# kan-bayashi/ParallelWaveGAN

Hardware: AMD Instinct MI355X
Metric: HiFi-GAN V1 22.05 kHz generator inference RTF^-1 (audio samples/s) (higher is better)
Workload: dtype f32; 1 GPU; HiFi-GAN V1 generator fwd, LJSpeech 22.05 kHz, B16 x 800 mel frames per GPU, fp32, random init; global_batch=16, parallelism=replicas x1

## Files before the change

### include/pwg_kernels.h

```cpp
#ifndef PWG_KERNELS_H_
#define PWG_KERNELS_H_

#include <stddef.h>
#include <stdint.h>

#ifdef __cplusplus
extern "C" {
#endif

typedef enum pwg_status {
  PWG_OK = 0,
  PWG_ERR_BAD_SHAPE = -1,
  PWG_ERR_UNSUPPORTED = -2,
  PWG_ERR_LAUNCH = -3,
  PWG_ERR_NULL = -4,
  PWG_ERR_WORKSPACE = -5
} pwg_status;

const char* pwg_last_error(void);
int pwg_abi_version(void);
int pwg_target_arch(void);

int pwg_prof_enable(int on);
int pwg_prof_reset(void);
// ... 48 lines not shown
  const float* g;
  float* scale;
  float* fwd;
  float* bwd;
  pwg_conv1d_desc desc;
} pwg_bank_item;
size_t pwg_weight_bank_table_bytes(int32_t n_items);
int pwg_weight_bank_build(const pwg_bank_item* items, int32_t n_items, void* table_host, size_t table_bytes,
                          int32_t* info);
int pwg_weight_bank_prepare(const void* table_dev, const int32_t* info, int32_t with_bwd, void* stream);

size_t pwg_conv1d_backward_data_workspace_floats(const pwg_conv1d_desc* d);
int pwg_conv1d_backward_data(const pwg_conv1d_desc* d, const float* dy, const float* w_packed_bwd,
                             const float* x, const float* accum, float* dx, float* workspace,
                             size_t workspace_floats, void* stream);
size_t pwg_conv1d_backward_weight_workspace_floats(const pwg_conv1d_desc* d);
int pwg_conv1d_backward_weight(const pwg_conv1d_desc* d, const float* x, const float* dy, float* dw,
                               float* db, float* workspace, size_t workspace_floats, void* stream);

size_t pwg_conv1d_backward_weight_wn_workspace_floats(const pwg_conv1d_desc* d);
int pwg_conv1d_backward_weight_wn(const pwg_conv1d_desc* d, const float* x, const float* dy, const float* v,
                                  const float* g, float* dv, float* dg, float* db, float* workspace,
                                  size_t workspace_floats, void* stream);

int pwg_conv1d_num_tile_configs(void);
int pwg_conv1d_forward_cfg(const pwg_conv1d_desc* d, const float* x, const float* w_packed,
                           const float* bias, const float* add1, const float* add2, float* y,
                           int32_t tile_config, int32_t use_dma, void* stream);

int pwg_conv1d_bf16_supported(const pwg_conv1d_desc* d);
size_t pwg_conv1d_bf16_packed_weight_bytes(const pwg_conv1d_desc* d);
int pwg_conv1d_bf16_pack_weight(const pwg_conv1d_desc* d, const float* w, const float* scale, void* w_packed,
                                void* stream);
int pwg_conv1d_bf16_forward(const pwg_conv1d_desc* d, const float* x, const void* w_packed, const float* bias,
                            const float* add1, const float* add2, float* y, float* workspace, size_t workspace_floats,
                            void* stream);
int pwg_conv1d_bf16_forward_cfg(const pwg_conv1d_desc* d, const float* x, const void* w_packed, const float* bias,
                                const float* add1, const float* add2, float* y, int32_t mfma_shape, void* stream);

int pwg_conv1d_split_supported(const pwg_conv1d_desc* d);
size_t pwg_conv1d_split_packed_weight_bytes(const pwg_conv1d_desc* d);
int pwg_conv1d_split_pack_weight(const pwg_conv1d_desc* d, const float* w, const float* scale, void* w_packed,
                                 void* stream);
int pwg_conv1d_split_forward(const pwg_conv1d_desc* d, const float* x, const void* w_packed, const float* bias,
                             const float* add1, const float* add2, float* y, float* workspace, size_t workspace_floats,
                             void* stream);
int pwg_conv1d_split_forward_cfg(const pwg_conv1d_desc* d, const float* x, const void* w_packed, const float* bias,
                                 const float* add1, const float* add2, float* y, int32_t mfma_shape, int32_t tile_mode,
                                 void* stream);
int pwg_conv1d_split_step_form(const pwg_conv1d_desc* d);
int pwg_conv1d_split_forward_step(const pwg_conv1d_desc* d, const float* x, const void* w_packed, const float* bias,
                                  const float* add1, const float* add2, float* y, int32_t mfma_shape, int32_t tile_mode,
                                  int32_t step_form, void* stream);

int pwg_convtr1d_split_supported(const pwg_conv1d_desc* d);
size_t pwg_convtr1d_split_packed_weight_bytes(const pwg_conv1d_desc* d);
int pwg_convtr1d_split_pack_weight(const pwg_conv1d_desc* d, const float* w, const float* scale, void* w_packed,
                                   void* stream);
int pwg_convtr1d_split_forward(const pwg_conv1d_desc* d, const float* x, const void* w_packed, const float* bias,
                               const float* add1, const float* add2, float* y, float* workspace,
                               size_t workspace_floats, void* stream);
int pwg_convtr1d_split_forward_cfg(const pwg_conv1d_desc* d, const float* x, const void* w_packed, const float* bias,
                                   const float* add1, const float* add2, float* y, int32_t mfma_shape,
                                   int32_t tile_mode, void* stream);

int pwg_conv1d_stream_supported(const pwg_conv1d_desc* d);
size_t pwg_conv1d_stream_hist_floats(const pwg_conv1d_desc* d);
int pwg_conv1d_stream_forward(const pwg_conv1d_desc* d, const float* x, const float* hist_in, float* hist_out,
                              const float* w_packed, const float* bias, const float* add1, const float* add2, float* y,
                              void* stream);

int pwg_conv1d_stream_bf16_supported(const pwg_conv1d_desc* d);
int pwg_conv1d_stream_bf16_forward(const pwg_conv1d_desc* d, const float* x, const float* hist_in, float* hist_out,
                                   const void* w_packed_bf16, const float* bias, const float* add1,
                                   const float* add2, float* y, void* stream);

int pwg_conv1d_stream_delayed_supported(const pwg_conv1d_desc* d, int32_t delay1, int32_t delay2);
int pwg_conv1d_stream_delayed_forward(const pwg_conv1d_desc* d, const float* x, const float* hist_in, float* hist_out,
                                      const float* w_packed, const float* bias, const float* add1,
                                      const float* add1_hist_in, float* add1_hist_out, int32_t delay1, const float* add2,
                                      const float* add2_hist_in, float* add2_hist_out, int32_t delay2, int32_t valid_lo,
                                      int32_t valid_hi, float* y, void* stream);

int pwg_conv1d_stream_bf16_delayed_supported(const pwg_conv1d_desc* d, int32_t delay1, int32_t delay2);
int pwg_conv1d_stream_bf16_delayed_forward(const pwg_conv1d_desc* d, const float* x, const float* hist_in,
                                           float* hist_out, const void* w_packed_bf16, const float* bias,
                                           const float* add1, const float* add1_hist_in, float* add1_hist_out,
                                           int32_t delay1, const float* add2, const float* add2_hist_in,
                                           float* add2_hist_out, int32_t delay2, int32_t valid_lo, int32_t valid_hi,
                                           float* y, void* stream);

int pwg_conv1d_stream_slots_forward(const pwg_conv1d_desc* d, const float* x, const float* hist_in, float* hist_out,
                                    const float* w_packed, const float* bias, const float* add1,
                                    const float* add1_hist_in, float* add1_hist_out, int32_t delay1, const float* add2,
                                    const float* add2_hist_in, float* add2_hist_out, int32_t delay2, const int32_t* slots,
                                    int32_t rate, int32_t delay, float* y, void* stream);
int pwg_conv1d_stream_slots_forward_bf16(const pwg_conv1d_desc* d, const float* x, const float* hist_in, float* hist_out,
                                         const void* w_packed_bf16, const float* bias, const float* add1,
                                         const float* add1_hist_in, float* add1_hist_out, int32_t delay1,
                                         const float* add2, const float* add2_hist_in, float* add2_hist_out,
                                         int32_t delay2, const int32_t* slots, int32_t rate, int32_t delay, float* y,
                                         void* stream);

int pwg_conv1d_stream_mirrored_supported(const pwg_conv1d_desc* d);
int pwg_conv1d_stream_mirrored_forward(const pwg_conv1d_desc* d, const float* x, const float* hist_in, float* hist_out,
                                       const float* w_packed, const float* bias, float* y, int32_t in_lo, int32_t in_hi,
// ... 325 lines not shown
```

### parallelwavegan_amd/_lib.py

```python
import ctypes
import os

_HERE = os.path.dirname(os.path.abspath(__file__))
LIB_PATH = os.environ.get("PWG_KERNEL_LIB") or os.path.join(_HERE, "libpwgkernels.so")

PWG_ACT_NONE, PWG_ACT_LEAKY_RELU, PWG_ACT_TANH, PWG_ACT_RELU = 0, 1, 2, 3
PWG_PAD_ZERO, PWG_PAD_REFLECT, PWG_PAD_REPLICATE = 0, 1, 2
ABI_VERSION = 15
SPECTRAL_NORM_SCRATCH_FLOATS = 257


class ConvDesc(ctypes.Structure):

    _fields_ = [
        ("batch", ctypes.c_int32),
        ("c_in", ctypes.c_int32),
        ("c_out", ctypes.c_int32),
        ("t_in", ctypes.c_int32),
        ("t_out", ctypes.c_int32),
        ("width", ctypes.c_int32),
        ("kernel", ctypes.c_int32),
        ("stride", ctypes.c_int32),
        ("dilation", ctypes.c_int32),
        ("pad_left", ctypes.c_int32),
# ... 59 lines not shown
        ("a", ctypes.c_void_p),
        ("b", ctypes.c_void_p),
        ("da", ctypes.c_void_p),
        ("db", ctypes.c_void_p),
        ("n", ctypes.c_int64),
        ("mode", ctypes.c_int32),
        ("slot", ctypes.c_int32),
        ("scale", ctypes.c_float),
        ("c", ctypes.c_float),
    ]


RED_MAX_ITEMS = 64

_lib = None
_vp = ctypes.c_void_p
_i32 = ctypes.c_int32
_i64 = ctypes.c_int64
_f32 = ctypes.c_float

SIGNATURES = {
    "pwg_last_error": (ctypes.c_char_p, []),
    "pwg_abi_version": (ctypes.c_int, []),
    "pwg_target_arch": (ctypes.c_int, []),
    "pwg_debug_poison_lds": (ctypes.c_int, [ctypes.c_int]),
    "pwg_set_concurrency_hint": (ctypes.c_float, [ctypes.c_float]),
    "pwg_prof_enable": (ctypes.c_int, [ctypes.c_int]),
    "pwg_prof_reset": (ctypes.c_int, []),
    "pwg_prof_num_kernels": (ctypes.c_int, []),
    "pwg_prof_get": (ctypes.c_int, [_i32, ctypes.c_char_p, ctypes.c_size_t, ctypes.POINTER(ctypes.c_double),
                                    ctypes.POINTER(ctypes.c_int64), ctypes.POINTER(ctypes.c_double),
                                    ctypes.POINTER(ctypes.c_double)]),
    "pwg_conv1d_packed_weight_floats": (ctypes.c_size_t, [ctypes.POINTER(ConvDesc)]),
    "pwg_conv1d_pack_weight": (ctypes.c_int, [ctypes.POINTER(ConvDesc), _vp, _vp, _vp, _vp]),
    "pwg_conv1d_forward_workspace_floats": (ctypes.c_size_t, [ctypes.POINTER(ConvDesc)]),
    "pwg_conv1d_forward": (ctypes.c_int, [ctypes.POINTER(ConvDesc), _vp, _vp, _vp, _vp, _vp, _vp, _vp, ctypes.c_size_t,
                                          _vp]),
    "pwg_conv1d_bf16_supported": (ctypes.c_int, [ctypes.POINTER(ConvDesc)]),
    "pwg_conv1d_bf16_packed_weight_bytes": (ctypes.c_size_t, [ctypes.POINTER(ConvDesc)]),
    "pwg_conv1d_bf16_pack_weight": (ctypes.c_int, [ctypes.POINTER(ConvDesc), _vp, _vp, _vp, _vp]),
    "pwg_conv1d_bf16_forward": (ctypes.c_int, [ctypes.POINTER(ConvDesc), _vp, _vp, _vp, _vp, _vp, _vp, _vp, ctypes.c_size_t,
                                               _vp]),
    "pwg_conv1d_bf16_forward_cfg": (ctypes.c_int, [ctypes.POINTER(ConvDesc), _vp, _vp, _vp, _vp, _vp, _vp, _i32, _vp]),
    "pwg_conv1d_split_supported": (ctypes.c_int, [ctypes.POINTER(ConvDesc)]),
    "pwg_conv1d_split_packed_weight_bytes": (ctypes.c_size_t, [ctypes.POINTER(ConvDesc)]),
    "pwg_conv1d_split_pack_weight": (ctypes.c_int, [ctypes.POINTER(ConvDesc), _vp, _vp, _vp, _vp]),
    "pwg_conv1d_split_forward": (ctypes.c_int, [ctypes.POINTER(ConvDesc), _vp, _vp, _vp, _vp, _vp, _vp, _vp,
                                                ctypes.c_size_t, _vp]),
    "pwg_conv1d_split_forward_cfg": (ctypes.c_int, [ctypes.POINTER(ConvDesc), _vp, _vp, _vp, _vp, _vp, _vp, _i32, _i32,
                                                    _vp]),
    "pwg_conv1d_split_step_form": (ctypes.c_int, [ctypes.POINTER(ConvDesc)]),
    "pwg_conv1d_split_forward_step": (ctypes.c_int, [ctypes.POINTER(ConvDesc), _vp, _vp, _vp, _vp, _vp, _vp, _i32, _i32,
                                                     _i32, _vp]),
    "pwg_convtr1d_split_supported": (ctypes.c_int, [ctypes.POINTER(ConvDesc)]),
    "pwg_convtr1d_split_packed_weight_bytes": (ctypes.c_size_t, [ctypes.POINTER(ConvDesc)]),
    "pwg_convtr1d_split_pack_weight": (ctypes.c_int, [ctypes.POINTER(ConvDesc), _vp, _vp, _vp, _vp]),
    "pwg_convtr1d_split_forward": (ctypes.c_int, [ctypes.POINTER(ConvDesc), _vp, _vp, _vp, _vp, _vp, _vp, _vp,
                                                  ctypes.c_size_t, _vp]),
    "pwg_convtr1d_split_forward_cfg": (ctypes.c_int, [ctypes.POINTER(ConvDesc), _vp, _vp, _vp, _vp, _vp, _vp, _i32, _i32,
                                                      _vp]),
    "pwg_conv1d_stream_supported": (ctypes.c_int, [ctypes.POINTER(ConvDesc)]),
    "pwg_conv1d_stream_hist_floats": (ctypes.c_size_t, [ctypes.POINTER(ConvDesc)]),
    "pwg_conv1d_stream_forward": (ctypes.c_int, [ctypes.POINTER(ConvDesc), _vp, _vp, _vp, _vp, _vp, _vp, _vp, _vp, _vp]),
    "pwg_conv1d_stream_bf16_supported": (ctypes.c_int, [ctypes.POINTER(ConvDesc)]),
    "pwg_conv1d_stream_bf16_forward": (ctypes.c_int, [ctypes.POINTER(ConvDesc), _vp, _vp, _vp, _vp, _vp, _vp, _vp, _vp,
                                                      _vp]),
    "pwg_conv1d_stream_delayed_supported": (ctypes.c_int, [ctypes.POINTER(ConvDesc), _i32, _i32]),
    "pwg_conv1d_stream_delayed_forward": (ctypes.c_int, [ctypes.POINTER(ConvDesc), _vp, _vp, _vp, _vp, _vp, _vp, _vp, _vp,
                                                         _i32, _vp, _vp, _vp, _i32, _i32, _i32, _vp, _vp]),
    "pwg_conv1d_stream_bf16_delayed_supported": (ctypes.c_int, [ctypes.POINTER(ConvDesc), _i32, _i32]),
    "pwg_conv1d_stream_bf16_delayed_forward": (ctypes.c_int, [ctypes.POINTER(ConvDesc), _vp, _vp, _vp, _vp, _vp, _vp, _vp,
                                                              _vp, _i32, _vp, _vp, _vp, _i32, _i32, _i32, _vp, _vp]),
    "pwg_conv1d_stream_slots_forward": (ctypes.c_int, [ctypes.POINTER(ConvDesc), _vp, _vp, _vp, _vp, _vp, _vp, _vp, _vp,
                                                       _i32, _vp, _vp, _vp, _i32, _vp, _i32, _i32, _vp, _vp]),
    "pwg_conv1d_stream_slots_forward_bf16": (ctypes.c_int, [ctypes.POINTER(ConvDesc), _vp, _vp, _vp, _vp, _vp, _vp, _vp,
                                                            _vp, _i32, _vp, _vp, _vp, _i32, _vp, _i32, _i32, _vp, _vp]),
    "pwg_conv1d_stream_mirrored_supported": (ctypes.c_int, [ctypes.POINTER(ConvDesc)]),
    "pwg_conv1d_stream_mirrored_forward": (ctypes.c_int, [ctypes.POINTER(ConvDesc), _vp, _vp, _vp, _vp, _vp, _vp, _i32,
                                                          _i32, _i32, _i32, _vp]),
    "pwg_conv1d_packed_weight_bwd_floats": (ctypes.c_size_t, [ctypes.POINTER(ConvDesc)]),
    "pwg_conv1d_pack_weight_bwd": (ctypes.c_int, [ctypes.POINTER(ConvDesc), _vp, _vp, _vp, _vp]),
    "pwg_weight_bank_table_bytes": (ctypes.c_size_t, [_i32]),
    "pwg_weight_bank_build": (ctypes.c_int, [ctypes.POINTER(BankItem), _i32, _vp, ctypes.c_size_t,
                                             ctypes.POINTER(ctypes.c_int32)]),
    "pwg_weight_bank_prepare": (ctypes.c_int, [_vp, ctypes.POINTER(ctypes.c_int32), _i32, _vp]),
    "pwg_conv1d_backward_data_workspace_floats": (ctypes.c_size_t, [ctypes.POINTER(ConvDesc)]),
    "pwg_conv1d_backward_data": (ctypes.c_int, [ctypes.POINTER(ConvDesc), _vp, _vp, _vp, _vp, _vp, _vp, ctypes.c_size_t,
                                                _vp]),
    "pwg_conv1d_backward_weight_workspace_floats": (ctypes.c_size_t, [ctypes.POINTER(ConvDesc)]),
    "pwg_conv1d_backward_weight": (ctypes.c_int, [ctypes.POINTER(ConvDesc), _vp, _vp, _vp, _vp, _vp, ctypes.c_size_t, _vp]),
    "pwg_conv1d_backward_weight_wn_workspace_floats": (ctypes.c_size_t, [ctypes.POINTER(ConvDesc)]),
    "pwg_conv1d_backward_weight_wn": (ctypes.c_int, [ctypes.POINTER(ConvDesc), _vp, _vp, _vp, _vp, _vp, _vp, _vp, _vp,
                                                     ctypes.c_size_t, _vp]),
    "pwg_conv1d_num_tile_configs": (ctypes.c_int, []),
    "pwg_conv1d_forward_cfg": (ctypes.c_int, [ctypes.POINTER(ConvDesc), _vp, _vp, _vp, _vp, _vp, _vp, _i32, _i32, _vp]),
    "pwg_conv1d_plan": (ctypes.c_int, [ctypes.POINTER(ConvDesc), _i32, ctypes.POINTER(_i32)]),
    "pwg_conv1d_backward_weight_plan": (ctypes.c_int, [ctypes.POINTER(ConvDesc), _i32, _i32, ctypes.POINTER(_i32)]),
    "pwg_debug_conv_tile_of_workgroup": (ctypes.c_int, [_i32, _i32, _i32, _i32, _i32, _i32, _i32, ctypes.POINTER(_i32)]),
    "pwg_resunit_supported": (ctypes.c_int, [ctypes.POINTER(ResUnitDesc)]),
    "pwg_resunit_profitable": (ctypes.c_int, [ctypes.POINTER(ResUnitDesc)]),
    "pwg_resunit_packed_weight_floats": (ctypes.c_size_t, [_i32, _i32]),
    "pwg_resunit_pack_weight": (ctypes.c_int, [_i32, _i32, _vp, _vp, _vp, _vp]),
    "pwg_resunit_forward": (ctypes.c_int, [ctypes.POINTER(ResUnitDesc), _vp, _vp, _vp, _vp, _vp, _vp, _vp, _vp]),
    "pwg_resunit_split_supported": (ctypes.c_int, [ctypes.POINTER(ResUnitDesc)]),
    "pwg_resunit_split_forward": (ctypes.c_int, [ctypes.POINTER(ResUnitDesc), _vp, _vp, _vp, _vp, _vp, _vp, _vp, _vp]),
    "pwg_resunit_split_forward_cfg": (ctypes.c_int, [ctypes.POINTER(ResUnitDesc), _vp, _vp, _vp, _vp, _vp, _vp, _vp, _i32,
# ... 146 lines not shown
```

### parallelwavegan_amd/csrc/conv1d_split.hip

```cpp
#include "mfma_conv.h"

namespace pwg {
namespace {

constexpr int PARTS = 3;

struct SplitArgs : MfmaConvArgs {
  int plane;
  long part_stride;
  float pre_mul;
  unsigned pre_mask;
  int wide_out;
};

static int split_geometry(const pwg_conv1d_desc* d, MfmaConvGeom* g) {
  return mfma_conv_geometry("conv1d_split", PARTS, false, d, g);
}

__device__ __forceinline__ float pre_activate(float v, float mul, unsigned mask) {
  const float n = __uint_as_float(__float_as_uint(v * mul) & mask);
  return v > 0.f ? v : n;
}

template <int NT, bool CHECKED>
// ... 247 lines not shown
conv1d_split_streamed_mfma_kernel(SplitArgs a) {
  constexpr int HL = 64 / TILE;
  constexpr int KSTEPS = KC / (8 * HL);
  constexpr int TM = WM * 32 / TILE, TN = WN * 32 / TILE;
  constexpr int NREG = TILE * TILE / 64;
  constexpr int WAVES_N = 4 / WAVES_M;
  constexpr int MT = WAVES_M * WM * 32, NT = WAVES_N * WN * 32;
  typedef typename Mfma<TILE>::acc_t acc_t;

  extern __shared__ __attribute__((aligned(16))) unsigned char smem[];
  __bf16* xs = reinterpret_cast<__bf16*>(smem);

  const MfmaConvTile c = mfma_conv_tile<TILE, MT, NT, WAVES_M, VEC>(a);

  const unsigned wrow = c.m0 + c.wave_m * (WM * 32) + c.r;
  bf16x8 wf[3];
  SplitStepId step{0, 0, 0};
  split_step_request(wf, a.w, a.part_stride, wrow + split_step_rows<TILE>(a.cin_chunks, a.m_pad, step, c.h));

  acc_t acc[TM][TN];
#pragma unroll
  for (int mi = 0; mi < TM; ++mi)
#pragma unroll
    for (int ni = 0; ni < TN; ++ni)
#pragma unroll
      for (int i = 0; i < NREG; ++i) acc[mi][ni][i] = 0.f;

  for (int chunk = 0; chunk < a.cin_chunks; ++chunk) {
    if (chunk) __syncthreads();
    stage_chunk<NT, VEC>(a, c, chunk, xs);
    __syncthreads();
#pragma unroll 1
    for (int s = 0; s < a.taps * KSTEPS; ++s) {
      const SplitStepId next = split_step_successor(step, a.cin_chunks, a.taps, KSTEPS);
      split_step_streamed<TILE, TM, TN, kConvRow, true>(
          wf, a.w, a.part_stride, wrow + split_step_rows<TILE>(a.cin_chunks, a.m_pad, step, c.h),
          wrow + split_step_rows<TILE>(a.cin_chunks, a.m_pad, next, c.h), xs,
          c.sh + c.wave_n * (WN * 32) + c.r + step.tap * a.dil, split_step_off<TILE>(step, c.h), a.plane, acc);
      step = next;
    }
  }

  const size_t out_base = (size_t)c.b * a.c_out * a.t_out;
  const int row0 = c.m0 + c.wave_m * (WM * 32) + c.r, col0 = c.q0 + c.wave_n * (WN * 32) + 4 * c.h;
  const bool full = c.m0 + MT <= a.m && c.q0 + NT <= a.nq;
  if (!a.wide_out)
    split_epilogue<TILE, TM, TN, false, false>(a, acc, row0, col0, out_base);
  else if (full)
    split_epilogue<TILE, TM, TN, true, true>(a, acc, row0, col0, out_base);
  else
    split_epilogue<TILE, TM, TN, true, false>(a, acc, row0, col0, out_base);
}

template <bool VEC, bool STREAMED>
struct Family {
  template <int TILE, int WM, int WN, int WAVES_M>
  struct K {
    static constexpr auto fn = STREAMED ? conv1d_split_streamed_mfma_kernel<TILE, WM, WN, WAVES_M, VEC>
                                        : conv1d_split_mfma_kernel<TILE, WM, WN, WAVES_M, VEC>;
  };
};

static void split_fill_args(SplitArgs* a, const pwg_conv1d_desc* d, const MfmaConvGeom& g, const MfmaConvPlan& p,
                            const float* x, const void* w_packed, const float* bias, const float* add1, const float* add2,
                            float* y) {
  mfma_conv_fill_args(a, d, g, x, w_packed, bias, add1, add2, y);
  a->plane = p.plane;
  a->part_stride = image_elems(g) / 8;
  a->pre_mul = d->pre_act == PWG_ACT_LEAKY_RELU ? d->pre_slope : (d->pre_act == PWG_ACT_RELU ? 0.0f : 1.0f);
  a->pre_mask = d->pre_act == PWG_ACT_RELU ? 0u : ~0u;
  a->wide_out = d->t_out % 4 == 0 && ((reinterpret_cast<uintptr_t>(y) | reinterpret_cast<uintptr_t>(add1) |
                                       reinterpret_cast<uintptr_t>(add2)) & 15u) == 0;
}

constexpr int kStepPlanDecides = 0, kStepResident = 1, kStepStreamed = 2;
constexpr int kStreamedMinTaps = 7, kStreamedMinChunks = 2;
static int split_step_form(const MfmaConvGeom& g) {
  if (!split_image_addressable(image_elems(g))) return kStepResident;
  return g.taps >= kStreamedMinTaps && g.cin_chunks >= kStreamedMinChunks ? kStepStreamed : kStepResident;
}

static int split_forward(const pwg_conv1d_desc* d, const float* x, const void* w_packed, const float* bias,
                         const float* add1, const float* add2, float* y, int mfma_shape, int tile_mode, int step_form,
                         hipStream_t stream) {
  MfmaConvGeom g;
  int rc = split_geometry(d, &g);
  if (rc != PWG_OK) return rc;
  PWG_REQUIRE(step_form >= kStepPlanDecides && step_form <= kStepStreamed, PWG_ERR_BAD_SHAPE,
              "conv1d_split: step_form = %d (0 = the plan decides, 1 = resident, 2 = streamed)", step_form);
  rc = mfma_conv_check_forward("conv1d_split", d, x, w_packed, y, mfma_shape, tile_mode);
  if (rc != PWG_OK) return rc;
  const MfmaConvPlan p = mfma_conv_plan(d, g, PARTS, tile_mode, x, add1, add2);
  PWG_REQUIRE(step_form != kStepStreamed || split_image_addressable(image_elems(g)), PWG_ERR_UNSUPPORTED,
              "conv1d_split: weight image too large for the streamed step");
  const bool streamed = (step_form == kStepPlanDecides ? split_step_form(g) : step_form) == kStepStreamed;
  SplitArgs a;
  split_fill_args(&a, d, g, p, x, w_packed, bias, add1, add2, y);
  maybe_poison_lds(stream);
  ProfScope prof(stream, "conv1d_split_mfma_kernel", p.flops, p.bytes);
  if (p.vec) {
    if (streamed)
      mfma_conv_launch<Family<true, true>::K>(p, mfma_shape, a, stream);
    else
      mfma_conv_launch<Family<true, false>::K>(p, mfma_shape, a, stream);
  } else {
    if (streamed)
      mfma_conv_launch<Family<false, true>::K>(p, mfma_shape, a, stream);
    else
      mfma_conv_launch<Family<false, false>::K>(p, mfma_shape, a, stream);
  }
  PWG_CHECK_LAUNCH("conv1d_split");
  return PWG_OK;
}

struct ConvtrArgs : SplitArgs {
  int phases, out_off;
};

static int convtr_geometry(const pwg_conv1d_desc* d, MfmaConvGeom* g) {
  PWG_REQUIRE(d != nullptr, PWG_ERR_NULL, "convtr1d_split: NULL descriptor");
  PWG_REQUIRE(d->transposed, PWG_ERR_UNSUPPORTED,
              "convtr1d_split: not a transposed convolution (a stride-1 Conv1d runs on conv1d_split)");
  return mfma_conv_geometry("convtr1d_split", PARTS, true, d, g);
}

template <int N>
__device__ __forceinline__ void convtr_finish(float out_mul, float out_div, int post_act, float post_slope, f32x4 (&v)[N],
                                              const f32x4& bias, bool has_bias, bool has1, bool has2,
                                              const f32x4 (&t1)[N], const f32x4 (&t2)[N]) {
  if (has_bias) {
#pragma unroll
    for (int k = 0; k < N; ++k) v[k] += bias;
  }
  if (has1) {
#pragma unroll
    for (int k = 0; k < N; ++k) v[k] += t1[k];
  }
  if (has2) {
#pragma unroll
    for (int k = 0; k < N; ++k) v[k] += t2[k];
  }
  if (out_mul != 1.0f) {
#pragma unroll
    for (int k = 0; k < N; ++k) v[k] *= out_mul;
  }
  if (out_div != 1.0f) {
#pragma unroll
    for (int k = 0; k < N; ++k) v[k] = v[k] / out_div;
  }
  if (post_act == PWG_ACT_LEAKY_RELU) {
// ... 160 lines not shown
  if (rc == PWG_OK) rc = mfma_conv_check_forward("convtr1d_split", d, x, w_packed, y, mfma_shape, tile_mode);
  if (rc != PWG_OK) return rc;
  PWG_REQUIRE((long)(g.nq + 256) * g.phases < (1L << 31), PWG_ERR_UNSUPPORTED, "convtr1d_split: output row too long");
  const MfmaConvPlan p = mfma_conv_plan(d, g, PARTS, tile_mode, x, add1, add2);
  ConvtrArgs a;
  split_fill_args(&a, d, g, p, x, w_packed, bias, add1, add2, y);
  a.phases = g.phases;
  a.out_off = g.out_off;
  a.wide_out = a.wide_out && g.phases % 4 == 0 && g.out_off % 4 == 0;
  maybe_poison_lds(stream);
  ProfScope prof(stream, "convtr1d_split_mfma_kernel", p.flops, p.bytes);
  if (p.vec)
    mfma_conv_launch<ConvtrFamily<true>::K>(p, mfma_shape, a, stream);
  else
    mfma_conv_launch<ConvtrFamily<false>::K>(p, mfma_shape, a, stream);
  PWG_CHECK_LAUNCH("convtr1d_split");
  return PWG_OK;
}

constexpr int kDefaultMfmaShape = 16;

}
}

using namespace pwg;

extern "C" int pwg_conv1d_split_supported(const pwg_conv1d_desc* d) {
  MfmaConvGeom g;
  return split_geometry(d, &g) == PWG_OK ? 1 : 0;
}

extern "C" size_t pwg_conv1d_split_packed_weight_bytes(const pwg_conv1d_desc* d) {
  MfmaConvGeom g;
  if (split_geometry(d, &g) != PWG_OK) return 0;
  return (size_t)PARTS * image_elems(g) * sizeof(__bf16);
}

extern "C" int pwg_conv1d_split_pack_weight(const pwg_conv1d_desc* d, const float* w, const float* scale, void* w_packed,
                                            void* stream) {
  MfmaConvGeom g;
  int rc = split_geometry(d, &g);
  if (rc != PWG_OK) return rc;
  PWG_REQUIRE(w && w_packed, PWG_ERR_NULL, "conv1d_split_pack_weight: NULL pointer");
  mfma_conv_pack<PARTS>(d, g, w, scale, w_packed, (hipStream_t)stream);
  PWG_CHECK_LAUNCH("conv1d_split_pack_weight");
  return PWG_OK;
}

extern "C" int pwg_conv1d_split_forward(const pwg_conv1d_desc* d, const float* x, const void* w_packed, const float* bias,
                                        const float* add1, const float* add2, float* y, float* workspace,
                                        size_t workspace_floats, void* stream) {
  (void)workspace;
  (void)workspace_floats;
  return split_forward(d, x, w_packed, bias, add1, add2, y, kDefaultMfmaShape, 0, kStepPlanDecides, (hipStream_t)stream);
}

extern "C" int pwg_conv1d_split_forward_cfg(const pwg_conv1d_desc* d, const float* x, const void* w_packed,
                                            const float* bias, const float* add1, const float* add2, float* y,
                                            int32_t mfma_shape, int32_t tile_mode, void* stream) {
  return split_forward(d, x, w_packed, bias, add1, add2, y, mfma_shape, tile_mode, kStepPlanDecides, (hipStream_t)stream);
}

extern "C" int pwg_conv1d_split_forward_step(const pwg_conv1d_desc* d, const float* x, const void* w_packed,
                                             const float* bias, const float* add1, const float* add2, float* y,
                                             int32_t mfma_shape, int32_t tile_mode, int32_t step_form, void* stream) {
  return split_forward(d, x, w_packed, bias, add1, add2, y, mfma_shape, tile_mode, step_form, (hipStream_t)stream);
}

extern "C" int pwg_conv1d_split_step_form(const pwg_conv1d_desc* d) {
  MfmaConvGeom g;
  if (split_geometry(d, &g) != PWG_OK) return 0;
  return split_step_form(g);
}

extern "C" int pwg_convtr1d_split_supported(const pwg_conv1d_desc* d) {
  MfmaConvGeom g;
  return convtr_geometry(d, &g) == PWG_OK ? 1 : 0;
}

extern "C" size_t pwg_convtr1d_split_packed_weight_bytes(const pwg_conv1d_desc* d) {
  MfmaConvGeom g;
  if (convtr_geometry(d, &g) != PWG_OK) return 0;
  return (size_t)PARTS * image_elems(g) * sizeof(__bf16);
}

extern "C" int pwg_convtr1d_split_pack_weight(const pwg_conv1d_desc* d, const float* w, const float* scale, void* w_packed,
                                              void* stream) {
  MfmaConvGeom g;
  int rc = convtr_geometry(d, &g);
  if (rc != PWG_OK) return rc;
  PWG_REQUIRE(w && w_packed, PWG_ERR_NULL, "convtr1d_split_pack_weight: NULL pointer");
  mfma_conv_pack<PARTS>(d, g, w, scale, w_packed, (hipStream_t)stream);
  PWG_CHECK_LAUNCH("convtr1d_split_pack_weight");
  return PWG_OK;
}

extern "C" int pwg_convtr1d_split_forward(const pwg_conv1d_desc* d, const float* x, const void* w_packed, const float* bias,
                                          const float* add1, const float* add2, float* y, float* workspace,
                                          size_t workspace_floats, void* stream) {
  (void)workspace;
  (void)workspace_floats;
  return convtr_forward(d, x, w_packed, bias, add1, add2, y, kDefaultMfmaShape, 0, (hipStream_t)stream);
}

extern "C" int pwg_convtr1d_split_forward_cfg(const pwg_conv1d_desc* d, const float* x, const void* w_packed,
                                              const float* bias, const float* add1, const float* add2, float* y,
                                              int32_t mfma_shape, int32_t tile_mode, void* stream) {
  return convtr_forward(d, x, w_packed, bias, add1, add2, y, mfma_shape, tile_mode, (hipStream_t)stream);
}
```

### parallelwavegan_amd/layers/conv.py

```python
import math
import os

import torch

from .. import functional as Fn
from .. import ops


class _ConvNd(torch.nn.Module):
    transposed = False
    width_mode = False
    explicit_pad_min_elems = 1 << 20
    fold_batch = {"0": False, "1": True}.get(os.environ.get("PWG_FOLD_BATCH", ""), True)
    fold_max_cols = int(os.environ.get("PWG_FOLD_MAX_COLS", 40))
    fold_min_weight_bytes = 4 << 20
    precision = "fp32"
    split_exact = {"0": False, "1": True}.get(os.environ.get("PWG_SPLIT_EXACT", ""), True)
    split_admit_all = False

    def __init__(self, in_channels, out_channels, kernel_size, stride=1, padding=0, dilation=1, groups=1,
                 bias=True, output_padding=0, pad_mode="zero"):
        super().__init__()
        if in_channels % groups or out_channels % groups:
            raise ValueError("in_channels and out_channels must be divisible by groups")
# ... 111 lines not shown
        if self.has_spectral_norm:
            return Fn.SpectralNormFn.apply(self.weight_orig, self.weight_u, self.weight_v, self.training,
                                           self.spectral_eps)
        return self.weight

    def effective_weight(self):
        with torch.no_grad():
            return self.weight_tensor().detach()

    def _param_state(self):
        ps = [self.raw_weight] + ([self.weight_g] if self.has_weight_norm else [])
        if self.has_spectral_norm:
            ps += [self.weight_u, self.weight_v]
        return tuple(ops.tensor_state(p) for p in ps)

    def _params_key(self):
        return (ops.cache_epoch(),) + self._param_state()

    def prepared(self):
        key = self._params_key()
        if self._cache_packed is None or self._cache_packed.key != key:
            desc = self.make_desc(1, self._probe_len())
            with torch.no_grad():
                if self.has_weight_norm:
                    v = self._w3(self.weight_v.detach())
                    scale = ops.weight_norm_scale(v, self.weight_g.detach().reshape(-1).contiguous())
                    self._cache_packed = Fn.PreparedWeights(key, v, scale, None, desc)
                else:
                    w = self._w3(self.effective_weight())
                    self._cache_packed = Fn.PreparedWeights(key, w, None, None, desc)
        return self._cache_packed

    def adopt_prepared(self, pw):
        self._cache_packed = pw

    def holds_current(self, pw):
        return self._cache_packed is pw and pw.key == self._params_key()

    def _packed(self, pack, cached):
        if self.has_spectral_norm and self.training:
            return pack(self.make_desc(1, self._probe_len()), self._w3(self.effective_weight()))
        return cached(self.prepared())

    def packed_weight(self):
        return self._packed(ops.pack_weight, lambda pw: pw.fwd)

    def packed_weight_bf16(self):
        return self._packed(ops.pack_weight_bf16, lambda pw: pw.bf16())

    def packed_weight_split(self):
        return self._packed(ops.pack_weight_split, lambda pw: pw.split())

    def _split_route(self, desc, needs_grad=False):
        return split_admitted(desc.c_in, desc.c_out, desc.kernel, desc.batch * desc.t_out, needs_grad,
                              self.split_exact, self.split_admit_all) and ops.conv1d_split_supported(desc)

    def packed_weight_split_transposed(self):
        return self._packed(ops.pack_weight_split_transposed, lambda pw: pw.split_transposed())

    def _upsample_split_route(self, desc, needs_grad=False):
        return (self.transposed
                and upsample_split_admitted(desc.c_in, desc.c_out, desc.kernel, desc.stride, desc.batch * desc.t_out,
                                            needs_grad, self.split_exact, self.split_admit_all)
                and ops.convtr1d_split_supported(desc))

    def bf16_capable(self):
        return not self.width_mode and ops.conv1d_bf16_supported(self.make_desc(1, self._probe_len()))

    @staticmethod
    def _w3(w):
        return w.reshape(w.shape[0], w.shape[1], -1).contiguous()

    def _probe_len(self):
        return self.kernel_size * self.dilation + self.stride + max(0, -self.padding_right)

    def geom(self):
        return dict(kernel=self.kernel_size, stride=self.stride, dilation=self.dilation, padding=self.padding,
                    padding_right=self.padding_right, groups=self.groups, transposed=self.transposed,
                    output_padding=self.output_padding, width=1, pad_mode=self.pad_mode)

    def out_length(self, t_in):
        raise NotImplementedError

    def make_desc(self, batch, t_in, width=1, **fused):
        raise NotImplementedError

    def _needs_grad(self, *tensors):
        if not torch.is_grad_enabled():
            return False
        if any(p.requires_grad for p in self.parameters(recurse=False)):
            return True
        return any(t is not None and t.requires_grad for t in tensors)

    def _fold_batch(self, x, add1, add2, precomputed):
        if not self.fold_batch or self.width_mode or self.transposed or x.dim() != 3 or self.pad_mode != "zero":
            return False
        if add1 is not None or add2 is not None or precomputed is not None:
            return False
        b, t_out = x.shape[0], self.out_length(x.shape[-1])
        w_bytes = 4 * self.out_channels * (self.in_channels // self.groups) * self.kernel_size
        return b >= 4 and 0 < t_out <= self.fold_max_cols and w_bytes >= self.fold_min_weight_bytes

    def forward(self, x, pre_act=None, pre_slope=0.0, post_act=None, post_slope=0.0, add1=None, add2=None,
                out_mul=1.0, out_div=1.0, precomputed=None):
        if self._fold_batch(x, add1, add2, precomputed):
            b, c, t = x.shape
            xf = x.permute(1, 2, 0).contiguous().view(1, c, t, b)
            y = self._forward(xf, b, pre_act, pre_slope, post_act, post_slope, None, None, out_mul, out_div, None)
# ... 26 lines not shown
            b = x.shape[0]
            if width_mode:
                h, width = x.shape[2], x.shape[3]
                desc = self.make_desc(b, h, width=width, **fused)
                y = ops.conv1d_forward(desc, x.reshape(b, x.shape[1], -1).contiguous(), self.packed_weight(),
                                       None if self.bias is None else self.bias.detach(),
                                       None if add1 is None else add1.reshape(b, self.out_channels, -1),
                                       None if add2 is None else add2.reshape(b, self.out_channels, -1))
                return y.reshape(b, self.out_channels, desc.t_out, width)
            if (self.pad_mode != "zero" and (self.padding > 0 or self.padding_right > 0) and not self.transposed
                    and x.numel() >= self.explicit_pad_min_elems):
                xp = Fn.pad1d(x, self.padding, self.padding_right, self.pad_mode)
                t_out = self.out_length(x.shape[-1])
                desc = ops.make_conv_desc(b, self.in_channels, self.out_channels, xp.shape[-1], t_out, self.kernel_size,
                                          self.stride, self.dilation, 0, self.groups, transposed=False, **fused)
                return ops.conv1d_forward(desc, xp, self.packed_weight(),
                                          None if self.bias is None else self.bias.detach(), add1, add2)
            desc = self.make_desc(b, x.shape[-1], **fused)
            if self.precision == "bf16" and ops.conv1d_bf16_supported(desc):
                return ops.conv1d_forward_bf16(desc, x.contiguous(), self.packed_weight_bf16(),
                                               None if self.bias is None else self.bias.detach(), add1, add2)
            if self.precision == "fp32" and self._split_route(desc):
                return ops.conv1d_forward_split(desc, x.contiguous(), self.packed_weight_split(),
                                                None if self.bias is None else self.bias.detach(), add1, add2)
            if self.precision == "fp32" and self._upsample_split_route(desc):
                return ops.conv1d_forward_split_transposed(desc, x.contiguous(), self.packed_weight_split_transposed(),
                                                           None if self.bias is None else self.bias.detach(), add1, add2)
            return ops.conv1d_forward(desc, x.contiguous(), self.packed_weight(),
                                      None if self.bias is None else self.bias.detach(), add1, add2)

    def extra_repr(self):
        norm = "weight_norm" if self.has_weight_norm else ("spectral_norm" if self.has_spectral_norm else "none")
        return (f"{self.in_channels}, {self.out_channels}, kernel_size={self.kernel_size}, stride={self.stride}, "
                f"padding={self.padding}, dilation={self.dilation}, groups={self.groups}, norm={norm}")


SPLIT_ADMITTED = {
    (128, 128, 7): 6400,
    (128, 128, 11): 6400,
    (256, 256, 7): 6400,
    (256, 256, 11): 6400,
}


def split_admitted(c_in, c_out, kernel, cols, needs_grad, enabled=True, admit_all=False):
    if needs_grad or not enabled:
        return False
    if admit_all:
        return True
    min_cols = SPLIT_ADMITTED.get((c_in, c_out, kernel))
    return min_cols is not None and cols >= min_cols


UPSAMPLE_SPLIT_MIN_COLS = 800
UPSAMPLE_SPLIT_ADMITTED = {
    (512, 256, 8): 102400,
    (256, 128, 8): 6400,
    (128, 64, 2): 12800,
    (64, 32, 2): 25600,
}


def upsample_split_admitted(c_in, c_out, kernel, stride, cols, needs_grad, enabled=True, admit_all=False):
    if needs_grad or not enabled or kernel != 2 * stride:
        return False
    if admit_all:
        return True
    min_cols = UPSAMPLE_SPLIT_ADMITTED.get((c_in, c_out, stride))
    return min_cols is not None and cols >= max(min_cols, UPSAMPLE_SPLIT_MIN_COLS)


RESUNIT_SPLIT_MIN_COLS = 20480
RESUNIT_SPLIT_ADMITTED = {
    (64, 3, True): ("unit", 20480),
    (64, 7, True): ("pair", 20480),
    (64, 11, True): ("pair", 20480),
    (32, 7, True): ("unit", 25600),
    (32, 11, True): ("unit", 25600),
}


def resunit_split_admitted(channels, kernel, has_conv2, cols, needs_grad, enabled=True, admit_all=False):
    if needs_grad or not enabled:
        return None
    if admit_all:
        return "unit"
    form, min_cols = RESUNIT_SPLIT_ADMITTED.get((channels, kernel, bool(has_conv2)), (None, 0))
    return form if form is not None and cols >= max(min_cols, RESUNIT_SPLIT_MIN_COLS) else None


def each_conv(module):
    return (m for m in module.modules() if isinstance(m, _ConvNd))


def group_image(owner, slot, convs, pack, *extra):
    key = extra + tuple(cv._params_key() for cv in convs)
    held = getattr(owner, slot, None)
    if held is None or held[0] != key:
        hs = [cv.prepared() for cv in convs]
        with torch.no_grad():
            held = (key, pack(*(t for h in hs for t in (h.w, h.scale))))
        setattr(owner, slot, held)
    return held[1]


def bf16_no_backward_error(module, model):
    return RuntimeError(
        f"{module.__class__.__name__} is in bf16 inference precision, which has no backward pass: run it under "
        f"torch.no_grad() ({model}.inference(..., precision='bf16') does), or switch back with "
        "utils.set_inference_precision(model, 'fp32') before training")


class Conv1d(_ConvNd):

    transposed = False

    def out_length(self, t_in):
        return ops.conv_out_length(t_in, self.kernel_size, self.stride, self.dilation, self.padding, self.padding_right)

    def make_desc(self, batch, t_in, width=1, **fused):
        return ops.make_conv_desc(batch, self.in_channels, self.out_channels, t_in, self.out_length(t_in),
                                  self.kernel_size, self.stride, self.dilation, self.padding, self.groups,
                                  transposed=False, width=width, pad_mode=self.pad_mode, **fused)


class Conv2d(Conv1d):

    width_mode = True

# ... 32 lines not shown
```

### parallelwavegan_amd/ops.py

```python
import ctypes

import torch

from . import _lib
from ._lib import ConvDesc, ResUnitDesc, WaveNetDesc

ACT = {None: _lib.PWG_ACT_NONE, "none": _lib.PWG_ACT_NONE, "leaky_relu": _lib.PWG_ACT_LEAKY_RELU,
       "tanh": _lib.PWG_ACT_TANH, "relu": _lib.PWG_ACT_RELU}
PAD = {"zero": _lib.PWG_PAD_ZERO, "reflect": _lib.PWG_PAD_REFLECT, "replicate": _lib.PWG_PAD_REPLICATE}


PARAM_EPOCH = [0]


def bump_param_epoch():
    PARAM_EPOCH[0] += 1


def cache_epoch():
    return PARAM_EPOCH[0]


def param_epoch(p):
    return getattr(p, "_pwg_epoch", 0)
# ... 163 lines not shown


def _conv1d_forward_mfma(kind, desc, image_desc, x, w_packed, bias, add1, add2, out, cfg, op="conv1d", entry="cfg"):
    name = f"{op}_forward_{kind}"
    _require_device(x, bias, add1, add2, out)
    if not w_packed.is_cuda or w_packed.dtype != torch.uint8:
        raise RuntimeError(f"{name}: w_packed must be the device image of pack_weight_{kind}")
    if out is None:
        out = torch.empty((desc.batch, desc.c_out, desc.t_out), device=x.device, dtype=torch.float32)
    assert x.numel() == desc.batch * desc.c_in * desc.t_in, (tuple(x.shape), desc.batch, desc.c_in, desc.t_in)
    assert out.numel() == desc.batch * desc.c_out * desc.t_out
    image_bytes = getattr(_lib.lib(), f"pwg_{op}_{kind}_packed_weight_bytes")(ctypes.byref(image_desc))
    if image_bytes == 0:
        _lib.check(-1, f"{op}_{kind}_packed_weight_bytes")
    assert w_packed.numel() == image_bytes, f"{name}: w_packed is not this layer's {kind} image"
    for t in (add1, add2):
        assert t is None or t.numel() == out.numel()
    args = (ctypes.byref(desc), _ptr(x), _ptr(w_packed), _ptr(bias), _ptr(add1), _ptr(add2), _ptr(out))
    if cfg is None:
        rc = getattr(_lib.lib(), f"pwg_{op}_{kind}_forward")(*args, None, 0, _stream())
    else:
        rc = getattr(_lib.lib(), f"pwg_{op}_{kind}_forward_{entry}")(*args, *cfg, _stream())
    _lib.check(rc, name)
    return out


def pack_weight_bf16(desc, w, scale=None):
    return _pack_weight_mfma("bf16", _zero_padded(desc), w, scale)


def conv1d_forward_bf16(desc, x, w_packed, bias=None, add1=None, add2=None, out=None, mfma_shape=None):
    return _conv1d_forward_mfma("bf16", desc, _zero_padded(desc), x, w_packed, bias, add1, add2, out,
                                None if mfma_shape is None else (int(mfma_shape),))


def conv1d_split_supported(desc):
    return bool(_lib.lib().pwg_conv1d_split_supported(ctypes.byref(desc)))


def pack_weight_split(desc, w, scale=None):
    return _pack_weight_mfma("split", desc, w, scale)


STEP_FORMS = {1: "resident", 2: "streamed"}


def conv1d_split_step_form(desc):
    form = _lib.lib().pwg_conv1d_split_step_form(ctypes.byref(desc))
    if form == 0:
        _lib.check(-1, "conv1d_split_step_form")
    return STEP_FORMS[form]


def conv1d_forward_split(desc, x, w_packed, bias=None, add1=None, add2=None, out=None, mfma_shape=None, tile_mode=0,
                         step_form=0):
    if step_form:
        cfg = (int(mfma_shape or 16), int(tile_mode), int(step_form))
        return _conv1d_forward_mfma("split", desc, desc, x, w_packed, bias, add1, add2, out, cfg, entry="step")
    cfg = None if mfma_shape is None and not tile_mode else (int(mfma_shape or 16), int(tile_mode))
    return _conv1d_forward_mfma("split", desc, desc, x, w_packed, bias, add1, add2, out, cfg)


def convtr1d_split_supported(desc):
    return bool(_lib.lib().pwg_convtr1d_split_supported(ctypes.byref(desc)))


def pack_weight_split_transposed(desc, w, scale=None):
    return _pack_weight_mfma("split", desc, w, scale, op="convtr1d")


def conv1d_forward_split_transposed(desc, x, w_packed, bias=None, add1=None, add2=None, out=None, mfma_shape=None,
                                    tile_mode=0):
    cfg = None if mfma_shape is None and not tile_mode else (int(mfma_shape or 16), int(tile_mode))
    return _conv1d_forward_mfma("split", desc, desc, x, w_packed, bias, add1, add2, out, cfg, op="convtr1d")


def conv1d_stream_supported(desc):
    return bool(_lib.lib().pwg_conv1d_stream_supported(ctypes.byref(desc)))


def conv1d_stream_hist_floats(desc):
    return _lib.lib().pwg_conv1d_stream_hist_floats(ctypes.byref(desc))


def _conv1d_stream_out(desc, x, hist_in, hist_out, add1, add2, out):
    if out is None:
        out = torch.empty((desc.batch, desc.c_out, desc.t_out), device=x.device, dtype=torch.float32)
    assert x.numel() == desc.batch * desc.c_in * desc.t_in, (tuple(x.shape), desc.batch, desc.c_in, desc.t_in)
    assert out.numel() == desc.batch * desc.c_out * desc.t_out
    n_hist = conv1d_stream_hist_floats(desc)
    for t in (hist_in, hist_out):
        assert t is None or t.numel() == n_hist, (tuple(t.shape), n_hist)
    for t in (add1, add2):
        assert t is None or t.numel() == out.numel()
    return out


def conv1d_stream_forward(desc, x, hist_in, hist_out, w_packed, bias=None, add1=None, add2=None, out=None):
    _require_device(x, hist_in, hist_out, w_packed, bias, add1, add2, out)
    out = _conv1d_stream_out(desc, x, hist_in, hist_out, add1, add2, out)
    _lib.check(_lib.lib().pwg_conv1d_stream_forward(ctypes.byref(desc), _ptr(x), _ptr(hist_in), _ptr(hist_out),
                                                    _ptr(w_packed), _ptr(bias), _ptr(add1), _ptr(add2), _ptr(out),
                                                    _stream()), "conv1d_stream_forward")
    return out


def conv1d_stream_delayed_supported(desc, delay1=0, delay2=0):
    return bool(_lib.lib().pwg_conv1d_stream_delayed_supported(ctypes.byref(desc), int(delay1), int(delay2)))
# ... 733 lines not shown
```

Baseline: 79.22 million samples/s.

## Add LDS-prefetched input-window split conv kernel and admit few-tap convs to split route

Adds a variant of the split-bf16 MFMA conv kernel that uses global_load_lds to fetch the next channel chunk's raw fp32 input window into LDS while the current chunk's MFMAs run. The goal is to overlap global loads with compute, at the cost of extra LDS per block. It is exposed through a new window_form API, but kWindowMaxTaps is 0, so the plan never picks it by default. Separately, the Python routing now sends 128- and 256-channel kernel-3 convs to the split path, and adds a 32-channel kernel-3 residual-unit split entry. Those routing changes do affect the default HiFi-GAN run.

```diff
diff --git a/include/pwg_kernels.h b/include/pwg_kernels.h
--- a/include/pwg_kernels.h
+++ b/include/pwg_kernels.h
@@ -124,6 +124,10 @@
 int pwg_conv1d_split_forward_step(const pwg_conv1d_desc* d, const float* x, const void* w_packed, const float* bias,
                                   const float* add1, const float* add2, float* y, int32_t mfma_shape, int32_t tile_mode,
                                   int32_t step_form, void* stream);
+int pwg_conv1d_split_window_form(const pwg_conv1d_desc* d);
+int pwg_conv1d_split_forward_window(const pwg_conv1d_desc* d, const float* x, const void* w_packed, const float* bias,
+                                    const float* add1, const float* add2, float* y, int32_t mfma_shape,
+                                    int32_t tile_mode, int32_t step_form, int32_t window_form, void* stream);
 
 int pwg_convtr1d_split_supported(const pwg_conv1d_desc* d);
 size_t pwg_convtr1d_split_packed_weight_bytes(const pwg_conv1d_desc* d);
diff --git a/parallelwavegan_amd/_lib.py b/parallelwavegan_amd/_lib.py
--- a/parallelwavegan_amd/_lib.py
+++ b/parallelwavegan_amd/_lib.py
@@ -135,6 +135,9 @@
     "pwg_conv1d_split_step_form": (ctypes.c_int, [ctypes.POINTER(ConvDesc)]),
     "pwg_conv1d_split_forward_step": (ctypes.c_int, [ctypes.POINTER(ConvDesc), _vp, _vp, _vp, _vp, _vp, _vp, _i32, _i32,
                                                      _i32, _vp]),
+    "pwg_conv1d_split_window_form": (ctypes.c_int, [ctypes.POINTER(ConvDesc)]),
+    "pwg_conv1d_split_forward_window": (ctypes.c_int, [ctypes.POINTER(ConvDesc), _vp, _vp, _vp, _vp, _vp, _vp, _i32,
+                                                       _i32, _i32, _i32, _vp]),
     "pwg_convtr1d_split_supported": (ctypes.c_int, [ctypes.POINTER(ConvDesc)]),
     "pwg_convtr1d_split_packed_weight_bytes": (ctypes.c_size_t, [ctypes.POINTER(ConvDesc)]),
     "pwg_convtr1d_split_pack_weight": (ctypes.c_int, [ctypes.POINTER(ConvDesc), _vp, _vp, _vp, _vp]),
diff --git a/parallelwavegan_amd/csrc/conv1d_split.hip b/parallelwavegan_amd/csrc/conv1d_split.hip
--- a/parallelwavegan_amd/csrc/conv1d_split.hip
+++ b/parallelwavegan_amd/csrc/conv1d_split.hip
@@ -323,6 +323,112 @@
     split_epilogue<TILE, TM, TN, true, false>(a, acc, row0, col0, out_base);
 }
 
+typedef __attribute__((address_space(3))) void* lds_ptr_t;
+
+static inline size_t split_raw_bytes(int rows) { return (size_t)KC * rows * sizeof(float); }
+
+__device__ __forceinline__ void request_raw_window(const float* __restrict__ xw, int t_in, int ngroups, float* raww,
+                                                   int lane) {
+  const int total = 8 * ngroups;
+  const int dq = 64 / ngroups, dr = 64 - dq * ngroups;
+  int j = lane / ngroups, g = lane - j * ngroups;
+  for (int e0 = 0; e0 < total; e0 += 64) {
+    if (e0 + lane < total)
+      __builtin_amdgcn_global_load_lds(xw + (size_t)j * t_in + 4 * g, (lds_ptr_t)(raww + e0 * 4), 16, 0, 0);
+    j += dq, g += dr;
+    if (g >= ngroups) g -= ngroups, ++j;
+  }
+}
+
+__device__ __forceinline__ void split_raw_window(const SplitArgs& a, const float* raww, int ngroups, __bf16* xs, int wave,
+                                                 int lane) {
+  for (int grp = lane; grp < ngroups; grp += 64) {
+    f32x4 st[8];
+#pragma unroll
+    for (int j = 0; j < 8; ++j) st[j] = *reinterpret_cast<const f32x4*>(raww + (j * ngroups + grp) * 4);
+#pragma unroll
+    for (int e = 0; e < 4; ++e) {
+      float v[8];
+#pragma unroll
+      for (int j = 0; j < 8; ++j) v[j] = pre_activate(st[j][e], a.pre_mul, a.pre_mask);
+      split3_store<8>(v, xs + (grp * 4 + e) * kConvRow + wave * 8, a.plane);
+      __builtin_amdgcn_sched_barrier(0);
+    }
+  }
+}
+
+template <int TILE, int WM, int WN, int WAVES_M>
+__global__ __launch_bounds__(256, WM * WN == 4 ? (TILE == 16 ? 3 : 2) : (WM * WN == 2 ? 3 : 4)) void
+conv1d_split_window_mfma_kernel(SplitArgs a) {
+  constexpr int HL = 64 / TILE;
+  constexpr int KSTEPS = KC / (8 * HL);
+  constexpr int TM = WM * 32 / TILE, TN = WN * 32 / TILE;
+  constexpr int NREG = TILE * TILE / 64;
+  constexpr int WAVES_N = 4 / WAVES_M;
+  constexpr int MT = WAVES_M * WM * 32, NT = WAVES_N * WN * 32;
+  typedef typename Mfma<TILE>::acc_t acc_t;
+
+  extern __shared__ __attribute__((aligned(16))) unsigned char smem[];
+  __bf16* xs = reinterpret_cast<__bf16*>(smem);
+
+  const MfmaConvTile c = mfma_conv_tile<TILE, MT, NT, WAVES_M, true>(a);
+  const int ngroups = (c.wcols + 3) >> 2;
+  float* raww = reinterpret_cast<float*>(xs + PARTS * a.plane) + c.wave * (8 * (a.plane / kConvRow));
+  const bool interior = c.base >= 0 && c.base + 4 * ngroups <= a.t_in;
+  const float* __restrict__ xw = c.xb + (size_t)(c.wave * 8) * a.t_in + c.base;
+  auto prefetched = [&](int chunk) { return interior && a.c_in - chunk * KC >= KC; };
+
+  if (prefetched(0)) request_raw_window(xw, a.t_in, ngroups, raww, c.lane);
+
+  acc_t acc[TM][TN];
+#pragma unroll
+  for (int mi = 0; mi < TM; ++mi)
+#pragma unroll
+    for (int ni = 0; ni < TN; ++ni)
+#pragma unroll
+      for (int i = 0; i < NREG; ++i) acc[mi][ni][i] = 0.f;
+
+  for (int chunk = 0; chunk < a.cin_chunks; ++chunk) {
+    if (chunk) __syncthreads();
+    if (prefetched(chunk)) {
+      asm volatile("s_waitcnt vmcnt(0)" ::: "memory");
+      split_raw_window(a, raww, ngroups, xs, c.wave, c.lane);
+    } else {
+      stage_chunk<NT, true>(a, c, chunk, xs);
+    }
+    __syncthreads();
+    if (chunk + 1 < a.cin_chunks && prefetched(chunk + 1))
+      request_raw_window(xw + (size_t)(chunk + 1) * KC * a.t_in, a.t_in, ngroups, raww, c.lane);
+    for (int tap = 0; tap < a.taps; ++tap) {
+#pragma unroll
+      for (int ks = 0; ks < KSTEPS; ++ks) {
+        const int oct = ks * HL + c.h;
+        const bf16x8* __restrict__ wp =
+            image_rows(a.w, a.cin_chunks, a.m_pad, tap, chunk, oct) + c.m0 + c.wave_m * (WM * 32) + c.r;
+        split_step<TILE, TM, TN, kConvRow, true>(wp, a.part_stride, xs, c.sh + c.wave_n * (WN * 32) + c.r + tap * a.dil,
+                                                 oct * 8, a.plane, acc);
+      }
+    }
+  }
+
+  const size_t out_base = (size_t)c.b * a.c_out * a.t_out;
+  const int row0 = c.m0 + c.wave_m * (WM * 32) + c.r, col0 = c.q0 + c.wave_n * (WN * 32) + 4 * c.h;
+  const bool full = c.m0 + MT <= a.m && c.q0 + NT <= a.nq;
+  if (!a.wide_out)
+    split_epilogue<TILE, TM, TN, false, false>(a, acc, row0, col0, out_base);
+  else if (full)
+    split_epilogue<TILE, TM, TN, true, true>(a, acc, row0, col0, out_base);
+  else
+    split_epilogue<TILE, TM, TN, true, false>(a, acc, row0, col0, out_base);
+}
+
+struct WindowFamily {
+  template <int TILE, int WM, int WN, int WAVES_M>
+  struct K {
+    static constexpr auto fn = conv1d_split_window_mfma_kernel<TILE, WM, WN, WAVES_M>;
+  };
+};
+
 template <bool VEC, bool STREAMED>
 struct Family {
   template <int TILE, int WM, int WN, int WAVES_M>
@@ -351,22 +457,62 @@
   return g.taps >= kStreamedMinTaps && g.cin_chunks >= kStreamedMinChunks ? kStepStreamed : kStepResident;
 }
 
+constexpr int kWindowPlanDecides = 0, kWindowStaged = 1, kWindowPrefetched = 2;
+constexpr size_t kLdsPerCu = 160 * 1024, kWindowLdsShare = kLdsPerCu / 3;
+constexpr int kWindowMaxTaps = 0;
+static size_t split_window_lds(const MfmaConvPlan& p) { return p.lds + split_raw_bytes(p.plane / kConvRow); }
+static bool split_window_covers(const MfmaConvPlan& p) { return p.vec && split_window_lds(p) <= kLdsPerCu; }
+static int split_window_form(const MfmaConvGeom& g, const MfmaConvPlan& p) {
+  if (!split_window_covers(p) || split_step_form(g) == kStepStreamed) return kWindowStaged;
+  return g.taps <= kWindowMaxTaps && g.cin_chunks >= 2 && split_window_lds(p) <= kWindowLdsShare ? kWindowPrefetched
+                                                                                                   : kWindowStaged;
+}
+
 static int split_forward(const pwg_conv1d_desc* d, const float* x, const void* w_packed, const float* bias,
                          const float* add1, const float* add2, float* y, int mfma_shape, int tile_mode, int step_form,
-                         hipStream_t stream) {
+                         int window_form, hipStream_t stream) {
   MfmaConvGeom g;
   int rc = split_geometry(d, &g);
   if (rc != PWG_OK) return rc;
   PWG_REQUIRE(step_form >= kStepPlanDecides && step_form <= kStepStreamed, PWG_ERR_BAD_SHAPE,
               "conv1d_split: step_form = %d (0 = the plan decides, 1 = resident, 2 = streamed)", step_form);
+  PWG_REQUIRE(window_form >= kWindowPlanDecides && window_form <= kWindowPrefetched, PWG_ERR_BAD_SHAPE,
+              "conv1d_split: window_form = %d (0 = the plan decides, 1 = staged, 2 = prefetched)", window_form);
   rc = mfma_conv_check_forward("conv1d_split", d, x, w_packed, y, mfma_shape, tile_mode);
   if (rc != PWG_OK) return rc;
   const MfmaConvPlan p = mfma_conv_plan(d, g, PARTS, tile_mode, x, add1, add2);
   PWG_REQUIRE(step_form != kStepStreamed || split_image_addressable(image_elems(g)), PWG_ERR_UNSUPPORTED,
               "conv1d_split: weight image too large for the streamed step");
-  const bool streamed = (step_form == kStepPlanDecides ? split_step_form(g) : step_form) == kStepStreamed;
+  PWG_REQUIRE(window_form != kWindowPrefetched || step_form != kStepStreamed, PWG_ERR_UNSUPPORTED,
+              "conv1d_split: the prefetched window (window_form = 2) has no streamed step (step_form = 2)");
+  PWG_REQUIRE(window_form != kWindowPrefetched || p.vec, PWG_ERR_UNSUPPORTED,
+              "conv1d_split: the prefetched window (window_form = 2) needs 16-B staging: t_in %% 4 == 0, x 16-B aligned, "
+              "a window of at most %d columns", 2 * p.nt);
+  PWG_REQUIRE(window_form != kWindowPrefetched || split_window_covers(p), PWG_ERR_UNSUPPORTED,
+              "conv1d_split: the prefetched window (window_form = 2) needs %zu B of LDS (> %zu)", split_window_lds(p),
+              kLdsPerCu);
+  const bool prefetched = window_form == kWindowPrefetched ||
+                          (window_form == kWindowPlanDecides && step_form == kStepPlanDecides &&
+                           split_window_form(g, p) == kWindowPrefetched);
+  const bool streamed = !prefetched && (step_form == kStepPlanDecides ? split_step_form(g) : step_form) == kStepStreamed;
   SplitArgs a;
   split_fill_args(&a, d, g, p, x, w_packed, bias, add1, add2, y);
+  if (prefetched) {
+    const size_t lds = split_window_lds(p);
+    void (*kern)(SplitArgs) = mfma_shape == 32 ? mfma_conv_tile_kernel<WindowFamily::K, 32, SplitArgs>(p)
+                                               : mfma_conv_tile_kernel<WindowFamily::K, 16, SplitArgs>(p);
+    if (lds > kConvMaxLds && !lds_limit_is_set(reinterpret_cast<const void*>(kern), lds)) {
+      hipError_t e = hipFuncSetAttribute(reinterpret_cast<const void*>(kern), hipFuncAttributeMaxDynamicSharedMemorySize,
+                                         (int)lds);
+      PWG_REQUIRE(e == hipSuccess, PWG_ERR_LAUNCH, "conv1d_split: cannot raise LDS limit to %zu: %s", lds,
+                  hipGetErrorString(e));
+    }
+    maybe_poison_lds(stream);
+    ProfScope prof(stream, "conv1d_split_mfma_kernel", p.flops, p.bytes);
+    hipLaunchKernelGGL(kern, p.grid, dim3(256), lds, stream, a);
+    PWG_CHECK_LAUNCH("conv1d_split");
+    return PWG_OK;
+  }
   maybe_poison_lds(stream);
   ProfScope prof(stream, "conv1d_split_mfma_kernel", p.flops, p.bytes);
   if (p.vec) {
@@ -633,19 +779,36 @@
                                         size_t workspace_floats, void* stream) {
   (void)workspace;
   (void)workspace_floats;
-  return split_forward(d, x, w_packed, bias, add1, add2, y, kDefaultMfmaShape, 0, kStepPlanDecides, (hipStream_t)stream);
+  return split_forward(d, x, w_packed, bias, add1, add2, y, kDefaultMfmaShape, 0, kStepPlanDecides, kWindowPlanDecides,
+                       (hipStream_t)stream);
 }
 
 extern "C" int pwg_conv1d_split_forward_cfg(const pwg_conv1d_desc* d, const float* x, const void* w_packed,
                                             const float* bias, const float* add1, const float* add2, float* y,
                                             int32_t mfma_shape, int32_t tile_mode, void* stream) {
-  return split_forward(d, x, w_packed, bias, add1, add2, y, mfma_shape, tile_mode, kStepPlanDecides, (hipStream_t)stream);
+  return split_forward(d, x, w_packed, bias, add1, add2, y, mfma_shape, tile_mode, kStepPlanDecides, kWindowPlanDecides,
+                       (hipStream_t)stream);
 }
 
 extern "C" int pwg_conv1d_split_forward_step(const pwg_conv1d_desc* d, const float* x, const void* w_packed,
                                              const float* bias, const float* add1, const float* add2, float* y,
                                              int32_t mfma_shape, int32_t tile_mode, int32_t step_form, void* stream) {
-  return split_forward(d, x, w_packed, bias, add1, add2, y, mfma_shape, tile_mode, step_form, (hipStream_t)stream);
+  return split_forward(d, x, w_packed, bias, add1, add2, y, mfma_shape, tile_mode, step_form, kWindowPlanDecides,
+                       (hipStream_t)stream);
+}
+
+extern "C" int pwg_conv1d_split_forward_window(const pwg_conv1d_desc* d, const float* x, const void* w_packed,
+                                               const float* bias, const float* add1, const float* add2, float* y,
+                                               int32_t mfma_shape, int32_t tile_mode, int32_t step_form,
+                                               int32_t window_form, void* stream) {
+  return split_forward(d, x, w_packed, bias, add1, add2, y, mfma_shape, tile_mode, step_form, window_form,
+                       (hipStream_t)stream);
+}
+
+extern "C" int pwg_conv1d_split_window_form(const pwg_conv1d_desc* d) {
+  MfmaConvGeom g;
+  if (split_geometry(d, &g) != PWG_OK) return 0;
+  return split_window_form(g, mfma_conv_plan(d, g, PARTS, 0, nullptr, nullptr, nullptr));
 }
 
 extern "C" int pwg_conv1d_split_step_form(const pwg_conv1d_desc* d) {
diff --git a/parallelwavegan_amd/layers/conv.py b/parallelwavegan_amd/layers/conv.py
--- a/parallelwavegan_amd/layers/conv.py
+++ b/parallelwavegan_amd/layers/conv.py
@@ -187,8 +187,9 @@
         return self._packed(ops.pack_weight_split, lambda pw: pw.split())
 
     def _split_route(self, desc, needs_grad=False):
-        return split_admitted(desc.c_in, desc.c_out, desc.kernel, desc.batch * desc.t_out, needs_grad,
-                              self.split_exact, self.split_admit_all) and ops.conv1d_split_supported(desc)
+        cls = (desc.c_in, desc.c_out, desc.kernel, desc.batch * desc.t_out, needs_grad, self.split_exact,
+               self.split_admit_all)
+        return (split_admitted(*cls) or split_fewtap_admitted(*cls)) and ops.conv1d_split_supported(desc)
 
     def packed_weight_split_transposed(self):
         return self._packed(ops.pack_weight_split_transposed, lambda pw: pw.split_transposed())
@@ -321,6 +322,22 @@
     return min_cols is not None and cols >= min_cols
 
 
+SPLIT_FEWTAP_MIN_COLS = 6400
+SPLIT_FEWTAP_ADMITTED = {
+    (128, 128, 3): 6400,
+    (256, 256, 3): 6400,
+}
+
+
+def split_fewtap_admitted(c_in, c_out, kernel, cols, needs_grad, enabled=True, admit_all=False):
+    if needs_grad or not enabled:
+        return False
+    if admit_all:
+        return True
+    min_cols = SPLIT_FEWTAP_ADMITTED.get((c_in, c_out, kernel))
+    return min_cols is not None and cols >= max(min_cols, SPLIT_FEWTAP_MIN_COLS)
+
+
 UPSAMPLE_SPLIT_MIN_COLS = 800
 UPSAMPLE_SPLIT_ADMITTED = {
     (512, 256, 8): 102400,
@@ -344,6 +361,7 @@
     (64, 3, True): ("unit", 20480),
     (64, 7, True): ("pair", 20480),
     (64, 11, True): ("pair", 20480),
+    (32, 3, True): ("unit", 51200),
     (32, 7, True): ("unit", 25600),
     (32, 11, True): ("unit", 25600),
 }
diff --git a/parallelwavegan_amd/ops.py b/parallelwavegan_amd/ops.py
--- a/parallelwavegan_amd/ops.py
+++ b/parallelwavegan_amd/ops.py
@@ -239,8 +239,21 @@
     return STEP_FORMS[form]
 
 
+WINDOW_FORMS = {1: "staged", 2: "prefetched"}
+
+
+def conv1d_split_window_form(desc):
+    form = _lib.lib().pwg_conv1d_split_window_form(ctypes.byref(desc))
+    if form == 0:
+        _lib.check(-1, "conv1d_split_window_form")
+    return WINDOW_FORMS[form]
+
+
 def conv1d_forward_split(desc, x, w_packed, bias=None, add1=None, add2=None, out=None, mfma_shape=None, tile_mode=0,
-                         step_form=0):
+                         step_form=0, window_form=0):
+    if window_form:
+        cfg = (int(mfma_shape or 16), int(tile_mode), int(step_form), int(window_form))
+        return _conv1d_forward_mfma("split", desc, desc, x, w_packed, bias, add1, add2, out, cfg, entry="window")
     if step_form:
         cfg = (int(mfma_shape or 16), int(tile_mode), int(step_form))
         return _conv1d_forward_mfma("split", desc, desc, x, w_packed, bias, add1, add2, out, cfg, entry="step")
```

Result: faster. 86.17 million samples/s, median of 6 (+8.8%).
